# ToughStoneX/Self-Supervised-MVS

Measured on AMD Instinct MI355X. Metric: depth-samples/sec (N=3, 640x512, D=192), higher is better.
Workload: dtype f32

## Files before the change

include/mvs_hip.h:

```cpp
#ifndef MVS_HIP_H
#define MVS_HIP_H

#ifdef __cplusplus
extern "C" {
#endif

#ifndef __HIP_PLATFORM_AMD__
typedef struct ihipStream_t* hipStream_t;
#endif

#define MVS_OK 0
#define MVS_ERR_SHAPE (-1)
#define MVS_ERR_UNSUPPORTED (-2)
#define MVS_ERR_LAUNCH (-3)
#define MVS_ERR_NULL (-4)
#define MVS_MAX_SRC 10

int mvs_version(void);
const char* mvs_last_error(void);
int mvs_is_emulation(void);
int mvs_launch_trace(char* buf, int cap);
int mvs_set_tuning(const char* key, int value);
int mvs_get_tuning(const char* key, int* value);

// ... 41 lines not shown
int mvs_convT3d_wgrad(const float* x, const float* gy, float* gw, float* ws, int B, int D, int H, int W, int Cin,
                      int Cout, int stride, hipStream_t stream);

#define MVS_UNET_MAX_BLOCKS 32
typedef struct MvsUnetBlock {
    int transposed, stride, src, skip;
    float eps, momentum;
    int cin, cout, d, h, w;
} MvsUnetBlock;
int mvs_unet_fwd(int n, const MvsUnetBlock* blocks, int B, const float* x, const float* const* w, const float* const* gamma,
                 const float* const* beta, float* const* running_mean, float* const* running_var, float* const* packed,
                 float* const* raw, float* const* y, float* const* stats, double* const* slots, const int* nslots,
                 const float* wprob, const float* bprob, int prob_cout, float* ws_prob, float* logits, hipStream_t stream);
int mvs_unet_bwd(int n, const MvsUnetBlock* blocks, int B, const float* x, const float* const* w, const float* wprob, int prob_cout,
                 const float* const* y, const float* const* raw, const float* const* stats, double* const* slots_b, const int* nslots,
                 float* const* packed_dgrad, const float* glogits, float* const* gbuf, float* const* draw, float* gx,
                 float* const* gw, float* const* wgrad_ws, float* const* dgamma, float* const* dbeta, hipStream_t main_stream,
                 hipStream_t side_stream, int join, int* side_stream_used);

int mvs_unet_time_wgrad(int block);
int mvs_unet_time_read(float* ms, int max_n);

long long mvs_conv3d_bf16_workspace_bytes(int Cin, int Cout, int stride, int transposed);
int mvs_conv3d_bf16_fwd(const void* x_bf16, const float* w, void* y, void* ws, int B, int D, int H, int W, int Cin, int Cout,
                        int stride, int transposed, const float* scale, const float* shift, const void* skip_bf16, int relu,
                        int out_is_f32, hipStream_t stream);
int mvs_cast_f32_bf16(const float* x, void* y_bf16, long long n, hipStream_t stream);

int mvs_bn_slots(int C);
int mvs_bn_stats_slots(const float* x, int G, long long Vg, int C, double* slots, int nslots, hipStream_t stream);
int mvs_bn_relu_fwd_slots(const float* x, const double* slots, int nslots, int G, long long Vg, int C, const float* gamma,
                          const float* beta, float eps, float momentum, float* running_mean, float* running_var,
                          const float* skip, int relu, float* stats, float* y, hipStream_t stream);
int mvs_bn_bwd_reduce_slots(const float* dy, const float* x, const float* stats, int relu, int G, long long Vg, int C,
                            double* slots, int nslots, hipStream_t stream);
int mvs_bn_relu_bwd_slots(const float* dy, const float* x, const float* stats, const double* slots, int nslots, int relu, int G,
                          long long Vg, int C, float* dx, float* dgamma, float* dbeta, hipStream_t stream);
int mvs_bn_eval_affine(const float* gamma, const float* beta, const float* running_mean, const float* running_var,
                       float eps, int C, float* scale, float* shift, hipStream_t stream);
int mvs_bn_relu_fwd(const float* x, const float* scale, const float* shift, const float* skip, int relu, long long V,
                    int C, float* y, hipStream_t stream);
int mvs_bn_frozen_stats(const float* gamma, const float* beta, const float* running_mean, const float* running_var, float eps,
                        int C, float* stats, hipStream_t stream);
int mvs_bn_relu_bwd_frozen(const float* dy, const float* raw, const float* stats, double* slots, int nslots, int have_sums,
                           int relu, long long V, int C, float* draw, float* dgamma, float* dbeta, hipStream_t stream);

int mvs_masked_smooth_l1_fwd(const float* est, const float* gt, const float* mask, long long n, float* out, hipStream_t stream);
int mvs_masked_smooth_l1_bwd(const float* est, const float* gt, const float* mask, const float* fwd_out, const float* gloss,
                             long long n, float* gest, hipStream_t stream);

long long mvs_depth_metrics_workspace_bytes(int B, int HW, int T);
int mvs_depth_metrics(const float* est, const float* gt, const void* mask, int mask_is_byte, const float* interval,
                      const float* thresholds, int T, int B, int HW, void* ws, float* out, float* per_image, double* meter,
                      long long* meter_count, hipStream_t stream);

long long mvs_sample_prep_workspace_bytes(int M, int H, int W);
int mvs_sample_prep(const void* src, int src_kind, long long src_image_stride, const float* params, const int* rect, float* imgs,
                    float* imgs_aug, float* imgs_seg, float* filter_mask, int mask_scale, int aug_center, int channels_last, int M,
                    int H, int W, void* ws, hipStream_t stream);

int mvs_adam_limits(int* chunk, int* max_segments);
int mvs_adam_step(float* p, const float* grad, float* m, float* v, long long n, int* step_counter, double lr, double beta1,
                  double beta2, double eps, double weight_decay, double grad_scale, hipStream_t stream);
int mvs_adam_step_table(float* p, float* m, float* v, long long n, const float* const* grads, const long long* offsets,
                        const long long* counts, int nseg, int* step_counter, double lr, double beta1, double beta2, double eps,
                        double weight_decay, double grad_scale, hipStream_t stream);
// ... 150 lines not shown
```

self-supervised-mvs_amd/_lib.py:

```python
from __future__ import annotations

import contextlib
import ctypes as C
import os

_HERE = os.path.dirname(os.path.abspath(__file__))
LIB_PATH = os.path.join(_HERE, "libmvs_hip.so")

_f = C.c_void_p
_i = C.c_int
_ll = C.c_longlong
_s = C.c_void_p
_fl = C.c_float

class MvsUnetBlock(C.Structure):
    _fields_ = [("transposed", _i), ("stride", _i), ("src", _i), ("skip", _i), ("eps", _fl), ("momentum", _fl),
                ("cin", _i), ("cout", _i), ("d", _i), ("h", _i), ("w", _i)]


class MvsFeatBlock(C.Structure):
    _fields_ = [("cin", _i), ("cout", _i), ("ks", _i), ("stride", _i), ("eps", _fl), ("momentum", _fl), ("w_channels_last", _i),
                ("h", _i), ("w", _i)]


# ... 26 lines not shown
    "mvs_refine_eval_fwd": (_i, [_i, _i, _i, _i, _i, _f, _ll, _f, _pp, _pp, _f, _f, _f, _f, _f, _f, _s]),
    "mvs_refine_bwd": (_i, [_i, _i, _i, _i, _i, _i, _pp, _f, _pp, _f, _pp, _f, _pp, C.POINTER(_i), _f, _f, _pp, _pp, _f, _f, _pp, _f, _pp, _pp, _f,
                            _f, _s]),
    "mvs_conv2d_dgrad_wl": (_i, [_f, _f, _f, _f, _i, _i, _i, _i, _i, _i, _i, _i, _s]),
    "mvs_conv2d_fwd_wl": (_i, [_f, _f, _f, _f, _f, _i, _i, _i, _i, _i, _i, _i, _i, _s]),
    "mvs_version": (_i, []),
    "mvs_last_error": (C.c_char_p, []),
    "mvs_is_emulation": (_i, []),
    "mvs_launch_trace": (_i, [C.c_char_p, _i]),
    "mvs_set_tuning": (_i, [C.c_char_p, _i]),
    "mvs_get_tuning": (_i, [C.c_char_p, C.POINTER(_i)]),
    "mvs_plane_sweep_variance_fwd": (_i, [_f, C.POINTER(C.c_void_p), _f, _f, _f, _i, _i, _i, _i, _i, _i, _i, _i, _i, _f, _s]),
    "mvs_plane_sweep_variance_fwd_bf16": (_i, [_f, C.POINTER(C.c_void_p), _f, _f, _f, _i, _i, _i, _i, _i, _i, _i, _i, _i, _f, _s]),
    "mvs_conv3d_bf16_workspace_bytes": (_ll, [_i] * 4),
    "mvs_conv3d_bf16_fwd": (_i, [_f, _f, _f, _f, _i, _i, _i, _i, _i, _i, _i, _i, _f, _f, _f, _i, _i, _s]),
    "mvs_cast_f32_bf16": (_i, [_f, _f, _ll, _s]),
    "mvs_plane_sweep_variance_bwd": (_i, [_f, _f, C.POINTER(C.c_void_p), _f, _f, _f, _i, _i, _i, _i, _i, _i, _i, _i, _i,
                                          _f, C.POINTER(C.c_void_p), _s]),
    "mvs_relative_projection": (_i, [_f, _f, _i, _i, _f, _f, _s]),
    "mvs_homo_warp_fwd": (_i, [_f, _f, _f, _f, _i, _i, _i, _i, _i, _i, _i, _f, _s]),
    "mvs_homo_warp_bwd": (_i, [_f, _f, _f, _f, _f, _i, _i, _i, _i, _i, _i, _i, _f, _s]),
    "mvs_conv3d_workspace_bytes": (_ll, [_i] * 8),
    "mvs_conv3d_pack_weights": (_i, [_i, _f, _f, _i, _i, _i, _i, _i, _i, _i, _s]),
    "mvs_conv3d_pack_weights_batch": (_i, [_i, C.POINTER(_i), C.POINTER(C.c_void_p), C.POINTER(C.c_void_p), C.POINTER(_i), _s]),
    "mvs_conv3d_fwd": (_i, [_f, _f, _f, _f, _i, _i, _i, _i, _i, _i, _i, _f, _f, _f, _i, _f, _i, _i, _s]),
    "mvs_conv3d_dgrad": (_i, [_f, _f, _f, _f, _f, _i, _i, _i, _i, _i, _i, _i, _f, _f, _f, _i, _i, _s]),
    "mvs_conv3d_wgrad": (_i, [_f, _f, _f, _f, _i, _i, _i, _i, _i, _i, _i, _s]),
    "mvs_convT3d_fwd": (_i, [_f, _f, _f, _f, _i, _i, _i, _i, _i, _i, _i, _f, _f, _f, _i, _f, _i, _i, _s]),
    "mvs_convT3d_dgrad": (_i, [_f, _f, _f, _f, _f, _i, _i, _i, _i, _i, _i, _i, _f, _f, _f, _i, _i, _s]),
    "mvs_convT3d_wgrad": (_i, [_f, _f, _f, _f, _i, _i, _i, _i, _i, _i, _i, _s]),
    "mvs_bn_slots": (_i, [_i]),
    "mvs_bn_stats_slots": (_i, [_f, _i, _ll, _i, _f, _i, _s]),
    "mvs_bn_relu_fwd_slots": (_i, [_f, _f, _i, _i, _ll, _i, _f, _f, _fl, _fl, _f, _f, _f, _i, _f, _f, _s]),
    "mvs_bn_finalize_slots": (_i, [_f, _i, _i, _ll, _i, _f, _f, _fl, _fl, _f, _f, _f, _s]),
    "mvs_bn_bwd_reduce_slots": (_i, [_f, _f, _f, _i, _i, _ll, _i, _f, _i, _s]),
    "mvs_bn_relu_bwd_slots": (_i, [_f, _f, _f, _f, _i, _i, _i, _ll, _i, _f, _f, _f, _s]),
    "mvs_bn_eval_affine": (_i, [_f, _f, _f, _f, _fl, _i, _f, _f, _s]),
    "mvs_bn_relu_fwd": (_i, [_f, _f, _f, _f, _i, _ll, _i, _f, _s]),
    "mvs_bn_frozen_stats": (_i, [_f, _f, _f, _f, _fl, _i, _f, _s]),
    "mvs_bn_relu_bwd_frozen": (_i, [_f, _f, _f, _f, _i, _i, _i, _ll, _i, _f, _f, _f, _s]),
    "mvs_masked_smooth_l1_fwd": (_i, [_f, _f, _f, _ll, _f, _s]),
    "mvs_masked_smooth_l1_bwd": (_i, [_f, _f, _f, _f, _f, _ll, _f, _s]),
    "mvs_depth_metrics_workspace_bytes": (_ll, [_i, _i, _i]),
    "mvs_depth_metrics": (_i, [_f, _f, _f, _i, _f, C.POINTER(_fl), _i, _i, _i, _f, _f, _f, _f, _f, _s]),
    "mvs_sample_prep_workspace_bytes": (_ll, [_i, _i, _i]),
    "mvs_sample_prep": (_i, [_f, _i, _ll, C.POINTER(_fl), C.POINTER(_i), _f, _f, _f, _f, _i, _i, _i, _i, _i, _i, _f, _s]),
    "mvs_adam_limits": (_i, [C.POINTER(_i), C.POINTER(_i)]),
    "mvs_adam_step": (_i, [_f, _f, _f, _f, _ll, _f] + [C.c_double] * 6 + [_s]),
    "mvs_adam_step_table": (_i, [_f, _f, _f, _ll, _pp, C.POINTER(_ll), C.POINTER(_ll), _i, _f] + [C.c_double] * 6 + [_s]),
    "mvs_softargmin_conf_fwd": (_i, [_f, _f, _i, _i, _i, _i, _i, _f, _f, _f, _f, _s]),
    "mvs_softargmin_conf_bwd": (_i, [_f, _f, _f, _i, _f, _f, _f, _i, _i, _i, _i, _f, _s]),
    "mvs_conv2d_workspace_floats": (_ll, [_i] * 8),
    "mvs_conv2d_fwd": (_i, [_f, _f, _f, _f, _f, _i, _i, _i, _i, _i, _i, _i, _s]),
    "mvs_conv2d_lrelu_fwd": (_i, [_f, _f, _f, _f, _f, _i, _i, _i, _i, _i, _i, _i, _fl, _s]),
    "mvs_conv2d_fwd_stats": (_i, [_f, _f, _f, _f, _f, _i, _i, _i, _i, _i, _i, _i, _i, _i, _i, _s]),
    "mvs_conv2d_pack_weights_batch": (_i, [_i, C.POINTER(C.c_void_p), C.POINTER(C.c_void_p), C.POINTER(_i), C.POINTER(_i), _s]),
    "mvs_conv2d_dgrad": (_i, [_f, _f, _f, _f, _i, _i, _i, _i, _i, _i, _i, _s]),
    "mvs_conv2d_dgrad_bnstats": (_i, [_f, _f, _f, _f, _i, _i, _i, _i, _i, _i, _f, _f, _f, _i, _i, _s]),
    "mvs_conv2d_wgrad": (_i, [_f, _f, _f, _f, _i, _i, _i, _i, _i, _i, _i, _s]),
    "mvs_conv2d_wgrad_batch_workspace_floats": (_ll, [_i, C.POINTER(_i)]),
    "mvs_conv2d_wgrad_batch": (_i, [_i, C.POINTER(C.c_void_p), C.POINTER(C.c_void_p), C.POINTER(C.c_void_p), _f, C.POINTER(_i), _s]),
    "mvs_conv2d_wgrad_batch_xf": (_i, [_i, C.POINTER(C.c_void_p), C.POINTER(C.c_void_p), _i, C.POINTER(C.c_void_p), C.POINTER(C.c_void_p), _f,
                                       C.POINTER(_i), _s]),
    "mvs_conv2d_fwd_stats_xf": (_i, [_f, _f, _f, _f, _f, _f, _i, _i, _i, _i, _i, _i, _i, _i, _i, _i, _s]),
    "mvs_depth_hypo_workspace_doubles": (_ll, [_i, _i, _i]),
    "mvs_depth_hypo": (_i, [_f, _f, _i, _i, _i, _f, _f, _s]),
# ... 68 lines not shown
        msg = self._mvs_last_error().decode("utf-8", "replace")
        if rc in (-1, -2, -4):
            raise ValueError("%s failed (%d): %s" % (name, rc, msg))
        raise RuntimeError("%s failed (%d): %s" % (name, rc, msg))

    def raw(self, name: str, *args):
        return getattr(self, "_" + name)(*args)

    def launch_trace(self):
        buf = C.create_string_buffer(4096)
        self._mvs_launch_trace(buf, len(buf))
        return [s for s in buf.value.decode().split(",") if s]

    def get_tuning(self, key: str) -> int:
        v = _i()
        self.call("mvs_get_tuning", key.encode(), C.byref(v))
        return v.value

    @contextlib.contextmanager
    def tuning(self, **knobs):
        old = []
        try:
            for key, val in knobs.items():
                old.append((key, self.get_tuning(key)))
                self.call("mvs_set_tuning", key.encode(), int(val))
            yield self
        finally:
            for key, val in reversed(old):
                self.call("mvs_set_tuning", key.encode(), val)


_INSTANCE = None

DEFAULT_TUNING = {"k8": 7, "xcd": 1, "side_pre": 1, "conv_pers": 1, "conv_pers_min": 1024, "conv_pers_nw": 8, "wgrad_pers": 1, "conv_small": 1, "tr2pw": 1, "sweep_bwd": 0, "wgrad_small": 0, "wgrad_groups": 768, "wgrad8_groups": 192, "wgrad8_gs": 2, "wgrad8_nch": 2, "cout1_h4": 1, "wgrad2d_batch": 2048, "sweep_fwd": 3}


def get() -> MvsLib:
    global _INSTANCE
    if _INSTANCE is None:
        _INSTANCE = MvsLib()
        for item in filter(None, os.environ.get("MVS_TUNING", "").split(",")):
            key, _, val = item.partition("=")
            DEFAULT_TUNING[key.strip()] = int(val)
            _INSTANCE.call("mvs_set_tuning", key.strip().encode(), int(val))
    return _INSTANCE


class KernelTimer:

    def __init__(self, only=None, names=None):
        self.only = only
        self.names = names
        self.events = {}

    def wants(self, name, tag):
        return self.only is None or name in self.only or tag in self.only

    def add(self, name, tag, ev0, ev1):
        self.events.setdefault((name, tag), []).append((ev0, ev1))

    _REG_NAMES = frozenset(("mvs_conv3d_fwd", "mvs_convT3d_fwd", "mvs_conv3d_dgrad", "mvs_convT3d_dgrad", "mvs_conv3d_wgrad", "mvs_convT3d_wgrad",
                            "mvs_bn_relu_fwd_slots", "mvs_bn_relu_bwd_slots", "mvs_bn_bwd_reduce_slots", "mvs_conv3d_pack_weights_batch"))

    def allows_c_entry(self, lib, blocks):
        if self.names is None:
            return False
        hit = self.names & self._REG_NAMES
# ... 57 lines not shown
```

self-supervised-mvs_amd/csrc/conv3d.hip:

```cpp
#include "mvs_rt.h"
#include "conv_map.h"

#include "conv_args.h"

__device__ __forceinline__ void conv_pack_weights_item(const float* __restrict__ w, float* __restrict__ wp, int geom, int CC,
                                                       int Cin, int Cout, int NB, int layout, int flip, int idx) {
    const int j = idx & 3, lane = (idx >> 2) & 63;
    const int nb = (idx >> 8) % NB, kk = (idx >> 8) / NB;
    const int co = nb * 16 + (lane & 15);
    int ks, chunk = 0, cls = 0;
    if (geom == GEOM_TR2_PW) {
        int k0 = 0;
        for (cls = 0; cls < 4; ++cls) {
            int n = tr2p_ntaps(cls) * CC / 16;
            if (kk < k0 + n) break;
            k0 += n;
        }
        ks = kk - k0;
        const int kf = 16 * ks + 4 * (lane >> 4) + j;
        const int tp = kf / CC, cip = kf % CC, n = lane & 15, pw = n >> 3, cop = n & 7;
        int dd, dh, dw, kd, kh;
        tr2p_tap(cls, tp, dd, dh, dw, kd, kh);
        int kw = tr2p_kw(pw, dw);
        float v = 0.f;
// ... 667 lines not shown
                float4 wv[3];
#pragma unroll
                for (int kh = 0; kh < 3; ++kh) wv[kh] = *reinterpret_cast<const float4*>(&wl[((kd * 3 + kh) * 3 + kw) * 8 + 4 * cq]);
#pragma unroll
                for (int r = 0; r < 6; ++r) {
                    const float4 xv = *reinterpret_cast<const float4*>(&tile[cq * NR * 4 + base + ((kd * CO1_RH + r) * CO1_RW + kw) * 4]);
#pragma unroll
                    for (int kh = 0; kh < 3; ++kh) {
                        const int o = r - kh;
                        if (o >= 0 && o < 4) {
                            acc[o] = fmaf(xv.x, wv[kh].x, acc[o]); acc[o] = fmaf(xv.y, wv[kh].y, acc[o]);
                            acc[o] = fmaf(xv.z, wv[kh].z, acc[o]); acc[o] = fmaf(xv.w, wv[kh].w, acc[o]);
                        }
                    }
                }
            }
    }
    const int qd = qd0 + pd, qw = qw0 + pw;
#pragma unroll
    for (int o4 = 0; o4 < 4; ++o4) {
        const int qh = qh0 + 4 * hg + o4;
        if (qd < a.QD && qh < a.QH && qw < a.QW) {
            const size_t o = (((size_t)b * a.Do + qd) * a.Ho + qh) * a.Wo + qw;
            float v = acc[o4];
            if (a.scale) v = v * a.scale[0] + a.shift[0];
            else if (a.shift) v = v + a.shift[0];
            if (a.relu) v = fmaxf(v, 0.f);
            if (a.skip) v += a.skip[o];
            a.y[o] = v;
        }
    }
}

template <int CX>
__global__ __launch_bounds__(256) void conv_wgrad_cg1_kernel(WgradArgs a) {
    using G = ConvGeom<GEOM_S1>;
    constexpr int CCP = CX + 1;
    constexpr int NR = G::RD * G::RH * G::RW;
    constexpr int NPOS = G::TQD * G::TQH * G::TQW;
    constexpr int NOUT = 27 * CX, OPT = (NOUT + 255) / 256;
    __shared__ float xt[NR * CCP];
    __shared__ float gt[NPOS];
    const int tid = threadIdx.x;
    float acc[OPT];
    int ooff[OPT];
#pragma unroll
    for (int k = 0; k < OPT; ++k) {
        acc[k] = 0.f;
        const int o = tid + 256 * k;
        const int tap = o < NOUT ? o / CX : 0, cx = o % CX;
        ooff[k] = (((tap / 9) * G::RH + (tap / 3) % 3) * G::RW + tap % 3) * CCP + cx;
    }
    const int ntiles = a.B * a.ntd * a.nth * a.ntw;
    for (int tile = blockIdx.x; tile < ntiles; tile += gridDim.x) {
        int t = tile;
        const int tw = t % a.ntw; t /= a.ntw;
        const int th = t % a.nth; t /= a.nth;
        const int td = t % a.ntd; t /= a.ntd;
        const int b = t;
        const int qd0 = td * G::TQD, qh0 = th * G::TQH, qw0 = tw * G::TQW;
        __syncthreads();
        {
            constexpr int XIT = (NR * (CX / 4) + 255) / 256;
            float4 xv[XIT];
            int xo[XIT];
            stage_load<XIT>(xv, xo, tid, NR * (CX / 4), [&](int i, const float*& src, int& o) {
// ... 932 lines not shown

extern "C" int mvs_conv3d_pack_weights_batch(int n, const int* ops, const float* const* w, float* const* ws, const int* shapes,
                                             hipStream_t stream) {
    MVS_REQUIRE(ops && w && ws && shapes, MVS_ERR_NULL, "conv3d_pack_weights_batch: null pointer argument");
    MVS_REQUIRE(n >= 0 && n <= 1024, MVS_ERR_SHAPE, "conv3d_pack_weights_batch: bad count %d", n);
    PackItem items[64];
    for (int i0 = 0; i0 < n; i0 += 64) {
        const int m = n - i0 < 64 ? n - i0 : 64;
        for (int i = 0; i < m; ++i) {
            const int* sh = shapes + (size_t)(i0 + i) * 7;
            MVS_REQUIRE(w[i0 + i] && ws[i0 + i], MVS_ERR_NULL, "conv3d_pack_weights_batch: null pointer in entry %d", i0 + i);
            IgemmPlan p;
            int rc = plan_for(ops[i0 + i], sh[0], sh[1], sh[2], sh[3], sh[4], sh[5], sh[6], p, "conv3d_pack_weights_batch");
            if (rc) return rc;
            rc = plan_pack(p, w[i0 + i], ws[i0 + i], items[i]);
            if (rc) return rc;
        }
        int rc = launch_pack(items, m, stream);
        if (rc) return rc;
    }
    return MVS_OK;
}

extern "C" int mvs_conv3d_fwd(const float* x, const float* w, float* y, float* ws, int B, int D, int H, int W,
                              int Cin, int Cout, int stride, const float* scale, const float* shift,
                              const float* skip, int relu, double* stat_slots, int nslots, int ws_packed, hipStream_t stream) {
    IgemmPlan p;
    int rc = plan_for(MVS_OP_CONV_FWD, B, D, H, W, Cin, Cout, stride, p, "conv3d_fwd");
    if (rc) return rc;
    Epilogue ep = {scale, shift, skip, relu, stat_slots, nslots, nullptr, nullptr};
    return run_igemm(p, x, w, y, ws, ep, ws_packed, stream);
}

extern "C" int mvs_conv3d_dgrad(const float* gy, const float* w, const float* add, float* gx, float* ws, int B, int D, int H, int W,
                                int Cin, int Cout, int stride, const float* bn_raw, const float* bn_stats, double* bn_slots,
                                int nslots, int ws_packed, hipStream_t stream) {
    IgemmPlan p;
    int rc = plan_for(MVS_OP_CONV_DGRAD, B, D, H, W, Cin, Cout, stride, p, "conv3d_dgrad");
    if (rc) return rc;
    Epilogue ep = {nullptr, nullptr, add, 0, bn_slots, nslots, bn_raw, bn_stats};
    MVS_REQUIRE(!bn_slots || bn_raw, MVS_ERR_NULL, "conv3d_dgrad: bn_slots without bn_raw");
    if (p.cin1) return run_cin1(p, gy, w, gx, ws, ep, ws_packed, stream);
    return run_igemm(p, gy, w, gx, ws, ep, ws_packed, stream);
}

extern "C" int mvs_conv3d_wgrad(const float* x, const float* gy, float* gw, float* ws, int B, int D, int H, int W,
                                int Cin, int Cout, int stride, hipStream_t stream) {
    int rc = check_stride(stride, D, H, W, "conv3d_wgrad");
    if (rc) return rc;
    return run_wgrad(stride == 2 ? GEOM_S2 : GEOM_S1, x, gy, gw, ws, B, D, H, W, Cin, Cout, stream);
}

extern "C" int mvs_convT3d_fwd(const float* x, const float* w, float* y, float* ws, int B, int D, int H, int W,
                               int Cin, int Cout, int stride, const float* scale, const float* shift,
                               const float* skip, int relu, double* stat_slots, int nslots, int ws_packed, hipStream_t stream) {
    IgemmPlan p;
    int rc = plan_for(MVS_OP_CONVT_FWD, B, D, H, W, Cin, Cout, stride, p, "convT3d_fwd");
    if (rc) return rc;
    Epilogue ep = {scale, shift, skip, relu, stat_slots, nslots, nullptr, nullptr};
    return run_igemm(p, x, w, y, ws, ep, ws_packed, stream);
}

extern "C" int mvs_convT3d_dgrad(const float* gy, const float* w, const float* add, float* gx, float* ws, int B, int D, int H,
                                 int W, int Cin, int Cout, int stride, const float* bn_raw, const float* bn_stats, double* bn_slots,
                                 int nslots, int ws_packed, hipStream_t stream) {
    IgemmPlan p;
// ... 15 lines not shown
```

self-supervised-mvs_amd/csrc/tuning.h:

```cpp
#pragma once

#define MVS_KNOBS(X) \
     \
    X(nt,               0,    0, 1,       "forward: non-temporal stores of the variance volume") \
    X(tile_w,           0,    0, 256,     "cached forward: pixel-tile width, 0 = the default tile") \
    X(dslab,            0,    0, 1 << 20, "forward: planes per workgroup, 0 = auto") \
    X(sweep_fwd,        3,    0, 4,       "forward: 0 taps through L1 every plane, 1 LDS-staged windows, 2 register-cached taps (4 ch/thread), 3 (8 ch/thread), 4 (16 ch/thread, <= 2 source views)") \
    X(sweep_bwd,        0,    0, 1,       "backward: 0 per-wave windows (<= 4 source views), 1 view-pair kernel with LDS atomics (what > 4 source views run)") \
    X(bwd_dslab,        0,    0, 1 << 20, "per-wave-window backward: planes per workgroup, 0 = auto") \
    X(bwd_nowin,        0,    0, 1,       "(tests) 1 = no LDS windows, every flush through global atomics") \
    X(bwd_cpt,          4,    4, 8,       "accepted and ignored (the 8-channels-per-thread backward was measured slower and removed)") \
    X(bwd_pf,           0,    0, 2,       "backward: 1 = block lookahead for 1-2 source views, 2 = ONE wave per SIMD for 3-4 source views") \
    X(bwd_gd,           2,    0, 2,       "backward: 2 = upstream gradient requested two planes ahead at 2 waves/SIMD (1-2 source views), 0 = rotating set at 3 waves/SIMD") \
    X(bwd_gd34,         0,    0, 1,       "backward: 3-4 source views with the upstream gradient requested two planes ahead (as 1-2 views run), 2 waves/SIMD") \
    X(fwd_pt,           0,    0, 1,       "cached forward with the per-wave projection table (plane_sweep_variance_fwd_pt_kernel): measured and rejected") \
    X(bwd_gpf,          0,    0, 1,       "per-wave-window backward requests the next planes' upstream gradient: 0 top of the group, 1 after the plane's gathers") \
    X(fwd_dl,           2,    0, 2,       "forward: 0 the round-1 loop, 1 LDS-staged per-plane depths, 2 + all views' re-gathers in flight before the first sample") \
    X(sweep_xcd,        0,    0, 1,       "XCD-compact workgroup order of the cached forward and the per-wave-window backward") \
     \
    X(conv_split,       1,    0, 1,       "0 keeps all Cout tiles in one workgroup") \
    X(conv_small,       1,    0, 2,       "quarter-size workgroup tiles for under-filled launches (0 never, 1 auto, 2 always)") \
    X(conv_small_wgs,   384,  0, 1 << 20, "... below this many workgroups (~1.5 per CU)") \
    X(tr2pw,            1,    0, 1,       "transposed stride-2 conv with Cout == 8 as W-parity-merged GEMMs (GEOM_TR2_PW)") \
    X(cc_wide,          0,    0, 1,       "quarter-tile kernels of the deep levels with all input channels as one chunk: measured and rejected") \
    X(cin1_vpt,         1,    1, 5,       "voxels per thread of the Cout == 1 layer's input gradient (4 = four from 1 M voxels on, 5 = always four): measured and rejected") \
    X(k8,               7,    0, 15,      "bit mask: 1|2 = Cout == 8 stride-1 layers run the 4x4x1 MFMA forward with the weights as the broadcast operand (0: generic kernel), +4 = weight gradient with g as the broadcast operand") \
    X(cout1_d4,         2,    0, 3,       "bit 1: the Cout = 1 layer of the bf16 inference path with four outputs per thread") \
    X(cout1_h4,         1,    0, 1,       "the 8 -> 1 layer with four outputs per thread (conv_cout1_h4_kernel); 0: one output per thread") \
    X(bf16_dp,          1,    0, 1,       "conv0 of the bf16 path (32 -> 8) with two output depth slices per MFMA (GEOM_S1_DP)") \
    X(xcd,              1,    0, 1,       "XCD-aware tile order in the broadcast-operand forward and the Cout == 8 weight gradient") \
    X(side_pre,         1,    0, 1,       "one-Cout-tile kernels with epilogue side inputs (skip / bn_raw) request them before the k-loop (1) or at the top of the epilogue (0)") \
    X(conv_pers,        1,    0, 1,       "one-chunk layers (16 -> <= 16, 8 -> 32 stride 1; 8 -> <= 16 stride 2) run the persistent kernels of conv3d_pers.hip") \
    X(conv_pers_min,    1024, 0, 1 << 30, "... when the one-tile kernel would launch at least this many workgroups (a persistent grid needs several tiles per workgroup)") \
    X(conv_pers_groups, 0,    0, 4096,    "workgroups of a persistent launch, 0 = what fits the GPU (tests: a few workgroups walk many tiles)") \
    X(conv_pers_nw,     8,    4, 8,       "waves per workgroup of conv_pers_kernel") \
    X(wgrad_pers,       1,    0, 1,       "one-chunk weight gradients run conv3d_pers.hip, from conv_pers_min tiles on") \
    X(wgrad_small,      0,    0, 3,       "quarter-size tiles in the generic weight-gradient kernel: 1 = 8-channel / stride-2 layers with many tiles, 2 = every layer with many tiles, 3 = always (tests)") \
    X(wgrad_groups,     768,  1, 768,     "persistent workgroups of the generic weight-gradient kernels") \
    X(wgrad8_groups,    192,  1, 512,     "... of the CG == 8 kernel (conv0)") \
    X(wgrad8_gs,        2,    0, 2,       "conv0's weight gradient in the output-gradient-shifted form on the 16x16x4 MFMA (conv_c8_wgrad_gs_kernel): 1 eight waves per workgroup, 2 sixteen; 0: conv_c8_wgrad_kernel (4x4x1 MFMA, X shifted)") \
    X(wgrad8_nch,       2,    1, 2,       "2 = the CG == 8 weight gradient stages both 16-channel chunks of a 32-channel X in one workgroup") \
    X(conv0_x3,         0,    0, 3,       "split-bf16 products (conv3d_x3.hip, opt-in): bit 0 = conv0's input gradient, bit 1 = conv0's forward") \
     \
    X(conv2d_pp,        1,    0, 1,       "3x3 stride-1 layers with <= 8 output channels as pixel-pair GEMMs (conv2d_igemm_kernel<.., PP>)") \
    X(conv2d_s2_mfma,   2,    0, 2,       "stride-2 input gradient: 2 ONE four-class MFMA pass with compacted taps, 1 four parity-class passes, 0 direct VALU form") \
    X(wgrad2d_groups,   256,  0, 1 << 20, "persistent workgroups of the weight gradient (used: 1 .. 1024; 256 = one per CU)") \
    X(wgrad2d_batch,    2048, 1, 4096,    "workgroups of the batched weight gradient (both launches together), shared out by work") \
     \
    X(c2w_tile,         0,    0, 2,       "0 = t128x64 when its launch has at least c2w_big_min workgroups, else t64x64; 1 = always t64x64; 2 = always t128x64") \
    X(c2w_big_min,      512,  0, 1 << 30, "... workgroups (two per CU)") \
    X(c2w_splitk,       0,    0, 8,       "K ranges of a layer: 0 = doubled (<= 8) while a t64x64 launch has fewer than c2w_split_min workgroups, 1 = never split, 2..8 = this many") \
    X(c2w_split_min,    512,  0, 1 << 30, "... workgroups (two per CU)") \
    X(c2w_bf_split_min, 2048, 0, 1 << 30, "c2w_split_min of the bf16 arms (arith = bf16): eight workgroups per CU")

struct MvsTuning {
#define MVS_KNOB_FIELD(key, def, lo, hi, doc) int key;
    MVS_KNOBS(MVS_KNOB_FIELD)
#undef MVS_KNOB_FIELD
};
extern MvsTuning g_tune;
```

self-supervised-mvs_amd/csrc/unet_pass.cpp:

```cpp
#include <string.h>
#include "mvs_rt.h"

#define MVS_UNET_MAX_BLOCKS 32
extern "C" {
struct MvsUnetBlock {
    int transposed, stride, src, skip;
    float eps, momentum;
    int cin, cout, d, h, w;
};
int mvs_conv3d_fwd(const float* x, const float* w, float* y, float* ws, int B, int D, int H, int W, int Cin, int Cout, int stride,
                   const float* scale, const float* shift, const float* skip, int relu, double* stat_slots, int nslots, int ws_packed,
                   hipStream_t stream);
int mvs_convT3d_fwd(const float* x, const float* w, float* y, float* ws, int B, int D, int H, int W, int Cin, int Cout, int stride,
                    const float* scale, const float* shift, const float* skip, int relu, double* stat_slots, int nslots, int ws_packed,
                    hipStream_t stream);
int mvs_conv3d_dgrad(const float* gy, const float* w, const float* add, float* gx, float* ws, int B, int D, int H, int W, int Cin, int Cout,
                     int stride, const float* bn_raw, const float* bn_stats, double* bn_slots, int nslots, int ws_packed, hipStream_t stream);
int mvs_convT3d_dgrad(const float* gy, const float* w, const float* add, float* gx, float* ws, int B, int D, int H, int W, int Cin, int Cout,
                      int stride, const float* bn_raw, const float* bn_stats, double* bn_slots, int nslots, int ws_packed, hipStream_t stream);
int mvs_conv3d_wgrad(const float* x, const float* gy, float* gw, float* ws, int B, int D, int H, int W, int Cin, int Cout, int stride,
                     hipStream_t stream);
int mvs_convT3d_wgrad(const float* x, const float* gy, float* gw, float* ws, int B, int D, int H, int W, int Cin, int Cout, int stride,
                      hipStream_t stream);
int mvs_bn_relu_fwd_slots(const float* x, const double* slots, int nslots, int G, long long Vg, int C, const float* gamma, const float* beta,
                          float eps, float momentum, float* running_mean, float* running_var, const float* skip, int relu, float* stats,
                          float* y, hipStream_t stream);
int mvs_bn_bwd_reduce_slots(const float* dy, const float* x, const float* stats, int relu, int G, long long Vg, int C, double* slots,
                            int nslots, hipStream_t stream);
int mvs_bn_relu_bwd_slots(const float* dy, const float* x, const float* stats, const double* slots, int nslots, int relu, int G, long long Vg,
                          int C, float* dx, float* dgamma, float* dbeta, hipStream_t stream);
}

#if defined(MVS_CPU_EMUL)
struct MvsForkJoin {
    void fork(hipStream_t, hipStream_t) {}
    void join(hipStream_t, hipStream_t) {}
};
#else
struct MvsForkJoin {
    static hipEvent_t event() {
        static thread_local hipEvent_t ev = nullptr;
        if (!ev) (void)hipEventCreateWithFlags(&ev, hipEventDisableTiming);
        return ev;
    }
    void fork(hipStream_t from, hipStream_t to) {
        hipEvent_t ev = event();
        (void)hipEventRecord(ev, from);
        (void)hipStreamWaitEvent(to, ev, 0);
    }
    void join(hipStream_t from, hipStream_t to) { fork(from, to); }
};
#endif

static int g_time_block = -2;
#if defined(MVS_CPU_EMUL)
extern "C" int mvs_unet_time_wgrad(int block) { g_time_block = block; return MVS_OK; }
extern "C" int mvs_unet_time_read(float*, int) { return 0; }
struct MvsBracket {
    MvsBracket(int, hipStream_t) {}
// ... 36 lines not shown
    }
};
#endif

#define MVS_TRY(expr)            \
    do {                         \
        const int rc_ = (expr);  \
        if (rc_) return rc_;     \
    } while (0)

static void out_dims(const MvsUnetBlock& b, int& d, int& h, int& w) {
    if (b.transposed && b.stride == 2) { d = 2 * b.d; h = 2 * b.h; w = 2 * b.w; }
    else if (b.stride == 2) { d = (b.d - 1) / 2 + 1; h = (b.h - 1) / 2 + 1; w = (b.w - 1) / 2 + 1; }
    else { d = b.d; h = b.h; w = b.w; }
}

static int check_program(int n, const MvsUnetBlock* blk, const char* what) {
    MVS_REQUIRE(n >= 1 && n <= MVS_UNET_MAX_BLOCKS && blk, MVS_ERR_SHAPE, "%s: 1..%d blocks, got %d", what, MVS_UNET_MAX_BLOCKS, n);
    for (int i = 0; i < n; ++i) {
        MVS_REQUIRE(blk[i].src >= -1 && blk[i].src < i && blk[i].skip >= -1 && blk[i].skip < i, MVS_ERR_SHAPE,
                    "%s: block %d reads block %d / adds block %d: a block may only use earlier blocks", what, i, blk[i].src, blk[i].skip);
        MVS_REQUIRE(blk[i].stride == 1 || blk[i].stride == 2, MVS_ERR_UNSUPPORTED, "%s: block %d has stride %d", what, i, blk[i].stride);
    }
    return MVS_OK;
}

extern "C" int mvs_unet_fwd(int n, const MvsUnetBlock* blk, int B, const float* x, const float* const* w, const float* const* gamma,
                            const float* const* beta, float* const* running_mean, float* const* running_var, float* const* packed,
                            float* const* raw, float* const* y, float* const* stats, double* const* slots, const int* nslots,
                            const float* wprob, const float* bprob, int prob_cout, float* ws_prob, float* logits, hipStream_t stream) {
    MVS_TRY(check_program(n, blk, "mvs_unet_fwd"));
    MVS_REQUIRE(x && w && gamma && beta && running_mean && running_var && packed && raw && y && stats && slots && nslots && wprob &&
                ws_prob && logits, MVS_ERR_NULL, "mvs_unet_fwd: null pointer argument");
    for (int i = 0; i < n; ++i) {
        const MvsUnetBlock& b = blk[i];
        const float* xin = b.src < 0 ? x : y[b.src];
        if (b.transposed)
            MVS_TRY(mvs_convT3d_fwd(xin, w[i], raw[i], packed[i], B, b.d, b.h, b.w, b.cin, b.cout, b.stride, nullptr, nullptr, nullptr, 0,
                                    slots[i], nslots[i], 1, stream));
        else
            MVS_TRY(mvs_conv3d_fwd(xin, w[i], raw[i], packed[i], B, b.d, b.h, b.w, b.cin, b.cout, b.stride, nullptr, nullptr, nullptr, 0,
                                   slots[i], nslots[i], 1, stream));
        int od, oh, ow;
        out_dims(b, od, oh, ow);
        MVS_TRY(mvs_bn_relu_fwd_slots(raw[i], slots[i], nslots[i], 1, (long long)B * od * oh * ow, b.cout, gamma[i], beta[i], b.eps,
                                      b.momentum, running_mean[i], running_var[i], b.skip >= 0 ? y[b.skip] : nullptr, 1, stats[i], y[i],
                                      stream));
    }
    int od, oh, ow;
    out_dims(blk[n - 1], od, oh, ow);
    return mvs_conv3d_fwd(y[n - 1], wprob, logits, ws_prob, B, od, oh, ow, blk[n - 1].cout, prob_cout, 1, nullptr, bprob, nullptr, 0, nullptr,
                          0, 0, stream);
}

extern "C" int mvs_unet_bwd(int n, const MvsUnetBlock* blk, int B, const float* x, const float* const* w, const float* wprob,
                            int prob_cout, const float* const* y, const float* const* raw, const float* const* stats,
                            double* const* slots_b, const int* nslots, float* const* packed_dgrad, const float* glogits,
                            float* const* gbuf, float* const* draw, float* gx, float* const* gw, float* const* wgrad_ws,
                            float* const* dgamma, float* const* dbeta, hipStream_t main_stream, hipStream_t side_stream, int join,
                            int* side_stream_used) {
    MVS_TRY(check_program(n, blk, "mvs_unet_bwd"));
    MVS_REQUIRE(x && w && wprob && y && raw && stats && slots_b && nslots && packed_dgrad && glogits && gbuf && draw && gw && wgrad_ws &&
                dgamma && dbeta, MVS_ERR_NULL, "mvs_unet_bwd: null pointer argument");
    MvsForkJoin fj;
    const bool async = side_stream != nullptr && side_stream != main_stream;
    bool side_used = false;
    auto wgrad = [&](int i, const float* xin, const float* gout, const MvsUnetBlock* b, int d, int h, int wd, int cin, int cout, int stride,
                     int transposed) -> int {
        (void)b;
        if (!gw[i]) return MVS_OK;
        hipStream_t st = main_stream;
        if (async) {
            fj.fork(main_stream, side_stream);
            st = side_stream;
            side_used = true;
        }
        MvsBracket br(i, st);
// ... 79 lines not shown
```

Measured before the change: 214.2.

## Fuse last block BatchNorm apply with the 8-to-1 probability convolution

Adds a kernel that finalizes BatchNorm statistics from the slots, applies the affine transform, ReLU and skip to the last UNet block, writes y, and computes the 8->1 3x3x3 probability convolution from a three-plane LDS ring in the same pass. This removes one separate launch and the re-read of y by the probability conv. Each workgroup handles a depth segment (head_seg) with halo recomputation. The costs are redundant slot reduction in every workgroup, one-wave workgroups, and halo planes loaded twice at segment boundaries.

```diff
diff --git a/include/mvs_hip.h b/include/mvs_hip.h
--- a/include/mvs_hip.h
+++ b/include/mvs_hip.h
@@ -97,6 +97,10 @@
 int mvs_bn_relu_fwd_slots(const float* x, const double* slots, int nslots, int G, long long Vg, int C, const float* gamma,
                           const float* beta, float eps, float momentum, float* running_mean, float* running_var,
                           const float* skip, int relu, float* stats, float* y, hipStream_t stream);
+int mvs_bn_relu_conv3d_cout1_fwd(const float* raw, const double* slots, int nslots, int B, int D, int H, int W, const float* gamma,
+                                 const float* beta, float eps, float momentum, float* running_mean, float* running_var,
+                                 const float* skip, float* stats, float* y, const float* wprob, const float* bprob, float* logits,
+                                 hipStream_t stream);
 int mvs_bn_bwd_reduce_slots(const float* dy, const float* x, const float* stats, int relu, int G, long long Vg, int C,
                             double* slots, int nslots, hipStream_t stream);
 int mvs_bn_relu_bwd_slots(const float* dy, const float* x, const float* stats, const double* slots, int nslots, int relu, int G,
diff --git a/self-supervised-mvs_amd/_lib.py b/self-supervised-mvs_amd/_lib.py
--- a/self-supervised-mvs_amd/_lib.py
+++ b/self-supervised-mvs_amd/_lib.py
@@ -82,6 +82,7 @@
     "mvs_bn_slots": (_i, [_i]),
     "mvs_bn_stats_slots": (_i, [_f, _i, _ll, _i, _f, _i, _s]),
     "mvs_bn_relu_fwd_slots": (_i, [_f, _f, _i, _i, _ll, _i, _f, _f, _fl, _fl, _f, _f, _f, _i, _f, _f, _s]),
+    "mvs_bn_relu_conv3d_cout1_fwd": (_i, [_f, _f, _i, _i, _i, _i, _i, _f, _f, _fl, _fl, _f, _f, _f, _f, _f, _f, _f, _f, _s]),
     "mvs_bn_finalize_slots": (_i, [_f, _i, _i, _ll, _i, _f, _f, _fl, _fl, _f, _f, _f, _s]),
     "mvs_bn_bwd_reduce_slots": (_i, [_f, _f, _f, _i, _i, _ll, _i, _f, _i, _s]),
     "mvs_bn_relu_bwd_slots": (_i, [_f, _f, _f, _f, _i, _i, _i, _ll, _i, _f, _f, _f, _s]),
@@ -216,7 +217,7 @@
 
 _INSTANCE = None
 
-DEFAULT_TUNING = {"k8": 7, "xcd": 1, "side_pre": 1, "conv_pers": 1, "conv_pers_min": 1024, "conv_pers_nw": 8, "wgrad_pers": 1, "conv_small": 1, "tr2pw": 1, "sweep_bwd": 0, "wgrad_small": 0, "wgrad_groups": 768, "wgrad8_groups": 192, "wgrad8_gs": 2, "wgrad8_nch": 2, "cout1_h4": 1, "wgrad2d_batch": 2048, "sweep_fwd": 3}
+DEFAULT_TUNING = {"k8": 7, "xcd": 1, "side_pre": 1, "conv_pers": 1, "conv_pers_min": 1024, "conv_pers_nw": 8, "wgrad_pers": 1, "conv_small": 1, "tr2pw": 1, "sweep_bwd": 0, "wgrad_small": 0, "wgrad_groups": 768, "wgrad8_groups": 192, "wgrad8_gs": 2, "wgrad8_nch": 2, "cout1_h4": 1, "head_fused": 1, "head_seg": 16, "wgrad2d_batch": 2048, "sweep_fwd": 3}
 
 
 def get() -> MvsLib:
diff --git a/self-supervised-mvs_amd/csrc/conv3d.hip b/self-supervised-mvs_amd/csrc/conv3d.hip
--- a/self-supervised-mvs_amd/csrc/conv3d.hip
+++ b/self-supervised-mvs_amd/csrc/conv3d.hip
@@ -723,6 +723,177 @@
     }
 }
 
+constexpr int PH_TH = 8, PH_TW = 32, PH_RH = PH_TH + 2, PH_RW = PH_TW + 2, PH_NV = PH_RH * PH_RW;
+constexpr int PH_NIT = (2 * PH_NV + 63) / 64;
+constexpr int PH_PLANE = 2 * PH_NV * 4;
+template <bool HAS_SKIP>
+__global__ __launch_bounds__(64) void bn_relu_conv_cout1_kernel(const float* __restrict__ raw, const float* __restrict__ skip,
+                                                                float* __restrict__ y, float* __restrict__ logits,
+                                                                const float* __restrict__ w, const float* __restrict__ bias,
+                                                                const double* __restrict__ slots, int nslots, double count,
+                                                                const float* __restrict__ gamma, const float* __restrict__ beta, float eps,
+                                                                float momentum, float* running_mean, float* running_var,
+                                                                float* __restrict__ stats, int D, int H, int W, int S, int nth, int ntw,
+                                                                int nseg) {
+    constexpr int C = 8;
+    __shared__ __attribute__((aligned(16))) float ring[3 * PH_PLANE];
+    __shared__ __attribute__((aligned(16))) float wl[27 * 8];
+    __shared__ double red[256];
+    __shared__ double tot[2 * C];
+    __shared__ __attribute__((aligned(16))) float aff[2 * C];
+    const int tid = threadIdx.x;
+    int t = blockIdx.x;
+    const int tw = t % ntw; t /= ntw;
+    const int th = t % nth; t /= nth;
+    const int sg = t % nseg; t /= nseg;
+    const int b = t;
+    const int h0 = th * PH_TH, w0 = tw * PH_TW, d0 = sg * S, dend = min(d0 + S, D);
+
+    const int cq = tid & 1;
+    int goff[PH_NIT], lofs[PH_NIT];
+    unsigned inside = 0, owned = 0;
+#pragma unroll
+    for (int k = 0; k < PH_NIT; ++k) {
+        const int i = tid + 64 * k;
+        const bool live = i < 2 * PH_NV;
+        const int vox = live ? i >> 1 : 0;
+        const int rh = vox / PH_RW, rw = vox % PH_RW;
+        const int ih = h0 + rh - 1, iw = w0 + rw - 1;
+        const bool in = live && ih >= 0 && ih < H && iw >= 0 && iw < W;
+        goff[k] = (min(max(ih, 0), H - 1) * W + min(max(iw, 0), W - 1)) * C + 4 * cq;
+        lofs[k] = live ? (cq * PH_NV + vox) * 4 : -1;
+        if (in) inside |= 1u << k;
+        if (in && rh >= 1 && rh <= PH_TH && rw >= 1 && rw <= PH_TW) owned |= 1u << k;
+    }
+    const size_t plane_stride = (size_t)H * W * C;
+    float4 rv[PH_NIT], kv[HAS_SKIP ? PH_NIT : 1];
+    auto issue = [&](int z) {
+        const size_t pb = ((size_t)b * D + min(max(z, 0), D - 1)) * plane_stride;
+#pragma unroll
+        for (int k = 0; k < PH_NIT; ++k) {
+            rv[k] = *reinterpret_cast<const float4*>(raw + pb + goff[k]);
+            if (HAS_SKIP) kv[HAS_SKIP ? k : 0] = *reinterpret_cast<const float4*>(skip + pb + goff[k]);
+        }
+    };
+
+    for (int i = tid; i < 27 * 8; i += 64) wl[i] = w[(size_t)(i % 8) * 27 + i / 8];
+    {
+        const int total = nslots * 2 * C;
+#pragma unroll
+        for (int m = 0; m < 4; ++m) {
+            const int t256 = tid + 64 * m;
+            double v[8];
+#pragma unroll
+            for (int j = 0; j < 8; ++j) {
+                const int idx = t256 + 256 * j;
+                v[j] = idx < total ? slots[idx] : 0.0;
+            }
+            double s = ((v[0] + v[1]) + (v[2] + v[3])) + ((v[4] + v[5]) + (v[6] + v[7]));
+            for (int idx = t256 + 2048; idx < total; idx += 256) s += slots[idx];
+            red[t256] = s;
+        }
+        __syncthreads();
+        if (tid < 2 * C) {
+            double s = 0.0;
+            for (int k = 0; k < 256 / (2 * C); ++k) s += red[k * 2 * C + tid];
+            tot[tid] = s;
+        }
+        __syncthreads();
+        if (tid < C) {
+            const double mean = tot[tid] / count;
+            double var = tot[C + tid] / count - mean * mean;
+            if (var < 0.0) var = 0.0;
+            if (blockIdx.x == 0 && running_mean) {
+                const double unbiased = count > 1.0 ? var * count / (count - 1.0) : var;
+                running_mean[tid] = (1.0f - momentum) * running_mean[tid] + momentum * (float)mean;
+                running_var[tid] = (1.0f - momentum) * running_var[tid] + momentum * (float)unbiased;
+            }
+            const float invstd = (float)(1.0 / sqrt(var + (double)eps));
+            const float sc = gamma[tid] * invstd, sh = beta[tid] - (float)mean * sc;
+            aff[tid] = sc;
+            aff[C + tid] = sh;
+            if (blockIdx.x == 0) { stats[tid] = (float)mean; stats[C + tid] = invstd; stats[2 * C + tid] = sc; stats[3 * C + tid] = sh; }
+        }
+        __syncthreads();
+    }
+    const float4 sc = *reinterpret_cast<const float4*>(aff + 4 * cq), sh = *reinterpret_cast<const float4*>(aff + C + 4 * cq);
+    const float bs = bias ? bias[0] : 0.f;
+
+    auto commit = [&](int z) {
+        const bool zin = z >= 0 && z < D;
+        float* __restrict__ pl = ring + ((z - d0 + 1) % 3) * PH_PLANE;
+        const unsigned in_z = zin ? inside : 0u;
+#pragma unroll
+        for (int k = 0; k < PH_NIT; ++k) {
+            float4 v = rv[k];
+            v.x = v.x * sc.x + sh.x; v.y = v.y * sc.y + sh.y; v.z = v.z * sc.z + sh.z; v.w = v.w * sc.w + sh.w;
+            v.x = fmaxf(v.x, 0.f); v.y = fmaxf(v.y, 0.f); v.z = fmaxf(v.z, 0.f); v.w = fmaxf(v.w, 0.f);
+            if (HAS_SKIP) {
+                const float4 s4 = kv[HAS_SKIP ? k : 0];
+                v.x += s4.x; v.y += s4.y; v.z += s4.z; v.w += s4.w;
+            }
+            if (!((in_z >> k) & 1u)) v = make_float4(0.f, 0.f, 0.f, 0.f);
+            if (lofs[k] >= 0) *reinterpret_cast<float4*>(pl + lofs[k]) = v;
+            rv[k] = v;
+        }
+    };
+    auto store_y = [&](int z) {
+        if (z < d0 || z >= dend) return;
+        const size_t pb = ((size_t)b * D + z) * plane_stride;
+#pragma unroll
+        for (int k = 0; k < PH_NIT; ++k)
+            if ((owned >> k) & 1u) *reinterpret_cast<float4*>(y + pb + goff[k]) = rv[k];
+    };
+    const int pw = tid & 31, hg = tid >> 5;
+    const int base = (4 * hg * PH_RW + pw) * 4;
+    float acc[4];
+    auto compute = [&](int zo) {
+        acc[0] = acc[1] = acc[2] = acc[3] = 0.f;
+#pragma unroll 1
+        for (int kdw = 0; kdw < 9; ++kdw) {
+            const int kd = kdw / 3, kw = kdw % 3;
+            const float* __restrict__ pl = ring + ((zo - d0 + kd) % 3) * PH_PLANE + base + kw * 4;
+#pragma unroll
+            for (int q = 0; q < 2; ++q) {
+                float4 wv[3];
+#pragma unroll
+                for (int kh = 0; kh < 3; ++kh) wv[kh] = *reinterpret_cast<const float4*>(&wl[((kd * 3 + kh) * 3 + kw) * 8 + 4 * q]);
+#pragma unroll
+                for (int r = 0; r < 6; ++r) {
+                    const float4 xv = *reinterpret_cast<const float4*>(&pl[(q * PH_NV + r * PH_RW) * 4]);
+#pragma unroll
+                    for (int kh = 0; kh < 3; ++kh) {
+                        const int o = r - kh;
+                        if (o >= 0 && o < 4) {
+                            acc[o] = fmaf(xv.x, wv[kh].x, acc[o]); acc[o] = fmaf(xv.y, wv[kh].y, acc[o]);
+                            acc[o] = fmaf(xv.z, wv[kh].z, acc[o]); acc[o] = fmaf(xv.w, wv[kh].w, acc[o]);
+                        }
+                    }
+                }
+            }
+        }
+    };
+    auto store_logits = [&](int zo) {
+        const int qw = w0 + pw;
+#pragma unroll
+        for (int o4 = 0; o4 < 4; ++o4) {
+            const int qh = h0 + 4 * hg + o4;
+            if (qh < H && qw < W) logits[(((size_t)b * D + zo) * H + qh) * W + qw] = bias ? acc[o4] + bs : acc[o4];
+        }
+    };
+    for (int z = d0 - 1; z <= dend; ++z) {
+        issue(z);
+        if (z - 2 >= d0) compute(z - 2);
+        MVS_WAVE_SYNC();
+        commit(z);
+        MVS_WAVE_SYNC();
+        store_y(z);
+        if (z - 2 >= d0) store_logits(z - 2);
+    }
+    compute(dend - 1);
+    store_logits(dend - 1);
+}
+
 template <int CX>
 __global__ __launch_bounds__(256) void conv_wgrad_cg1_kernel(WgradArgs a) {
     using G = ConvGeom<GEOM_S1>;
@@ -1721,6 +1892,29 @@
     return run_igemm(p, x, w, y, ws, ep, ws_packed, stream);
 }
 
+extern "C" int mvs_bn_relu_conv3d_cout1_fwd(const float* raw, const double* slots, int nslots, int B, int D, int H, int W,
+                                            const float* gamma, const float* beta, float eps, float momentum, float* running_mean,
+                                            float* running_var, const float* skip, float* stats, float* y, const float* wprob,
+                                            const float* bprob, float* logits, hipStream_t stream) {
+    MVS_REQUIRE(raw && slots && gamma && beta && stats && y && wprob && logits, MVS_ERR_NULL, "bn_relu_conv3d_cout1_fwd: null pointer argument");
+    MVS_REQUIRE(B >= 1 && D >= 1 && H >= 1 && W >= 1 && (long long)H * W * 8 < (1ll << 31) && nslots >= 1 && nslots <= 256 &&
+                (nslots & (nslots - 1)) == 0, MVS_ERR_SHAPE, "bn_relu_conv3d_cout1_fwd: bad shape %d x %d x %d x %d, slots=%d", B, D, H, W, nslots);
+    MVS_REQUIRE((running_mean == nullptr) == (running_var == nullptr), MVS_ERR_NULL,
+                "bn_relu_conv3d_cout1_fwd: running_mean and running_var go together");
+    const int S = g_tune.head_seg < D ? g_tune.head_seg : D;
+    const int nseg = mvs_cdiv(D, S), nth = mvs_cdiv(H, PH_TH), ntw = mvs_cdiv(W, PH_TW);
+    const long long nwg = (long long)B * nseg * nth * ntw;
+    MVS_REQUIRE(nwg < (1ll << 31), MVS_ERR_SHAPE, "bn_relu_conv3d_cout1_fwd: %lld workgroups", nwg);
+    const double count = (double)((long long)B * D * H * W);
+    if (skip)
+        MVS_LAUNCH((bn_relu_conv_cout1_kernel<true>), dim3((unsigned)nwg), dim3(64), 0, stream, raw, skip, y, logits, wprob, bprob, slots, nslots,
+                   count, gamma, beta, eps, momentum, running_mean, running_var, stats, D, H, W, S, nth, ntw, nseg);
+    else
+        MVS_LAUNCH((bn_relu_conv_cout1_kernel<false>), dim3((unsigned)nwg), dim3(64), 0, stream, raw, skip, y, logits, wprob, bprob, slots, nslots,
+                   count, gamma, beta, eps, momentum, running_mean, running_var, stats, D, H, W, S, nth, ntw, nseg);
+    return mvs_check_launch("bn_relu_conv_cout1");
+}
+
 extern "C" int mvs_conv3d_dgrad(const float* gy, const float* w, const float* add, float* gx, float* ws, int B, int D, int H, int W,
                                 int Cin, int Cout, int stride, const float* bn_raw, const float* bn_stats, double* bn_slots,
                                 int nslots, int ws_packed, hipStream_t stream) {
diff --git a/self-supervised-mvs_amd/csrc/tuning.h b/self-supervised-mvs_amd/csrc/tuning.h
--- a/self-supervised-mvs_amd/csrc/tuning.h
+++ b/self-supervised-mvs_amd/csrc/tuning.h
@@ -27,7 +27,9 @@
     X(k8,               7,    0, 15,      "bit mask: 1|2 = Cout == 8 stride-1 layers run the 4x4x1 MFMA forward with the weights as the broadcast operand (0: generic kernel), +4 = weight gradient with g as the broadcast operand") \
     X(cout1_d4,         2,    0, 3,       "bit 1: the Cout = 1 layer of the bf16 inference path with four outputs per thread") \
     X(cout1_h4,         1,    0, 1,       "the 8 -> 1 layer with four outputs per thread (conv_cout1_h4_kernel); 0: one output per thread") \
-    X(bf16_dp,          1,    0, 1,       "conv0 of the bf16 path (32 -> 8) with two output depth slices per MFMA (GEOM_S1_DP)") \
+    X(head_fused,       1,    0, 1,       "bit 0: mvs_unet_fwd runs the last block's BatchNorm apply (+ skip) and the 8 -> 1 prob convolution as ONE kernel (bn_relu_conv_cout1_kernel)") \
+    X(head_seg,         16,   1, 1 << 20, "... depth planes per workgroup of that kernel") \
+    X(bf16_dp,         1,    0, 1,       "conv0 of the bf16 path (32 -> 8) with two output depth slices per MFMA (GEOM_S1_DP)") \
     X(xcd,              1,    0, 1,       "XCD-aware tile order in the broadcast-operand forward and the Cout == 8 weight gradient") \
     X(side_pre,         1,    0, 1,       "one-Cout-tile kernels with epilogue side inputs (skip / bn_raw) request them before the k-loop (1) or at the top of the epilogue (0)") \
     X(conv_pers,        1,    0, 1,       "one-chunk layers (16 -> <= 16, 8 -> 32 stride 1; 8 -> <= 16 stride 2) run the persistent kernels of conv3d_pers.hip") \
diff --git a/self-supervised-mvs_amd/csrc/unet_pass.cpp b/self-supervised-mvs_amd/csrc/unet_pass.cpp
--- a/self-supervised-mvs_amd/csrc/unet_pass.cpp
+++ b/self-supervised-mvs_amd/csrc/unet_pass.cpp
@@ -25,6 +25,9 @@
 int mvs_bn_relu_fwd_slots(const float* x, const double* slots, int nslots, int G, long long Vg, int C, const float* gamma, const float* beta,
                           float eps, float momentum, float* running_mean, float* running_var, const float* skip, int relu, float* stats,
                           float* y, hipStream_t stream);
+int mvs_bn_relu_conv3d_cout1_fwd(const float* raw, const double* slots, int nslots, int B, int D, int H, int W, const float* gamma,
+                                 const float* beta, float eps, float momentum, float* running_mean, float* running_var, const float* skip,
+                                 float* stats, float* y, const float* wprob, const float* bprob, float* logits, hipStream_t stream);
 int mvs_bn_bwd_reduce_slots(const float* dy, const float* x, const float* stats, int relu, int G, long long Vg, int C, double* slots,
                             int nslots, hipStream_t stream);
 int mvs_bn_relu_bwd_slots(const float* dy, const float* x, const float* stats, const double* slots, int nslots, int relu, int G, long long Vg,
@@ -127,6 +130,7 @@
     MVS_TRY(check_program(n, blk, "mvs_unet_fwd"));
     MVS_REQUIRE(x && w && gamma && beta && running_mean && running_var && packed && raw && y && stats && slots && nslots && wprob &&
                 ws_prob && logits, MVS_ERR_NULL, "mvs_unet_fwd: null pointer argument");
+    const bool head_fused = (g_tune.head_fused & 1) && g_tune.cout1_h4 && blk[n - 1].cout == 8 && prob_cout == 1;
     for (int i = 0; i < n; ++i) {
         const MvsUnetBlock& b = blk[i];
         const float* xin = b.src < 0 ? x : y[b.src];
@@ -138,6 +142,9 @@
                                    slots[i], nslots[i], 1, stream));
         int od, oh, ow;
         out_dims(b, od, oh, ow);
+        if (i == n - 1 && head_fused)
+            return mvs_bn_relu_conv3d_cout1_fwd(raw[i], slots[i], nslots[i], B, od, oh, ow, gamma[i], beta[i], b.eps, b.momentum, running_mean[i],
+                                                running_var[i], b.skip >= 0 ? y[b.skip] : nullptr, stats[i], y[i], wprob, bprob, logits, stream);
         MVS_TRY(mvs_bn_relu_fwd_slots(raw[i], slots[i], nslots[i], 1, (long long)B * od * oh * ow, b.cout, gamma[i], beta[i], b.eps,
                                       b.momentum, running_mean[i], running_var[i], b.skip >= 0 ? y[b.skip] : nullptr, 1, stats[i], y[i],
                                       stream));
```

Result: no change. 216.3 (median of 6 runs) (+1.0%).
